# llGuy/madrona_renderer

Measured on AMD Instinct MI355X. Metric: rendered views/sec (whole node), N worlds x 64x64 RGB+depth, higher is better.
Workload: dtype f32

## Files before the change

madrona_renderer_amd/csrc/raster.hip:

```cpp
#include <hip/hip_runtime.h>
#include <algorithm>
#include <cstdlib>

#include "raster.hpp"
#include "raster_dev.hpp"

namespace mrx {
namespace {

constexpr int kWavesPerBlock = 4;
constexpr int kChunk = 64;
constexpr int kHot = 16;
constexpr int kBandRows = 16;
constexpr int kBlocksPerBand = 16;

struct WaveLds {
    float hot[kChunk][kHot];
    float cold[kChunk][kCold];
};

struct TileCtx {
    uint32_t view, tileX0, tileY0;
    uint32_t triBegin, numTris;
    int lx, ly;
// ... 185 lines not shown
                    resolvePixel<IDS>(p, L, bid[b], best[b], pxf[b & 7],
                                      (b >> 3) ? py1 : py0, outRgba[b], outId[b]);
        } else {
            for (uint32_t chunk = 0; chunk < t.numTris; chunk += kChunk) {
                const uint64_t mask = setupChunk<PV>(p, vc, t, chunk, lane, L, pr, lt);
                rasterBandBrute(L, mask, pxf, py0, py1, invNear, best, bid);
#pragma unroll
                for (int b = 0; b < kBlocksPerBand; ++b) {
                    if (bid[b] >= 0)
                        resolvePixel<IDS>(p, L, bid[b], best[b], pxf[b & 7],
                                          (b >> 3) ? py1 : py0, outRgba[b], outId[b]);
                    bid[b] = -1;
                }
                waveLdsSync();
            }
        }

#pragma unroll
        for (int b = 0; b < kBlocksPerBand; ++b) {
            const int r = b >> 3, bx = b & 7;
            const uint32_t fx = t.tileX0 + bx * 8 + t.lx;
            const uint32_t fy = t.tileY0 + band * kBandRows + r * 8 + t.ly;
            if (fx < p.nfast && fy < p.nslow) {
                const bool hit = best[b] > p.invFar;
                const float dep = hit ? 1.0f / best[b] : 0.0f;
                const size_t o = ((size_t)t.view * p.nslow + fy) * p.nfast + fx;
                if (storesRgb<OUT>(p.rgb))
                    p.rgb[o] = outRgba[b];
                if (storesDepth<OUT>(p.depth))
                    p.depth[o] = dep;
                if (IDS)
                    p.ids[o] = outId[b];
            }
        }
    }
}

template <bool IDS, bool MULTI, int OUT = kOutRGBD>
__global__ __launch_bounds__(kWave *kWavesPerBlock)
void rasterBruteKernel(const RasterParams p)
{
    bruteKernelBody<IDS, MULTI, OUT, false>(p);
}

template <bool IDS, bool MULTI>
__global__ __launch_bounds__(kWave *kWavesPerBlock)
void rasterBruteKernelPV(const RasterParams p)
{
    bruteKernelBody<IDS, MULTI, kOutByPointer, true>(p);
}

constexpr uint32_t kNearFree = 1u << 16;

template <int S0, int S1>
__device__ __forceinline__ uint32_t classifyStrips(const TriPlanes &c, uint32_t tileX0,
                                                   uint32_t tileY0, float invNear, float invFar,
                                                   bool &nearOk)
{
    const float X0 = (float)tileX0, Y0 = (float)tileY0;
    const float xa0 = c.A0 < 0.0f ? X0 : X0 + 31.0f;
    const float xa1 = c.A1 < 0.0f ? X0 : X0 + 31.0f;
    const float xa2 = c.A2 < 0.0f ? X0 : X0 + 31.0f;
    const float xdh = c.Dx < 0.0f ? X0 : X0 + 31.0f;
    const float xdl = c.Dx < 0.0f ? X0 + 31.0f : X0;
    const float yb0 = c.B0 < 0.0f ? Y0 : Y0 + 7.0f;
    const float yb1 = c.B1 < 0.0f ? Y0 : Y0 + 7.0f;
    const float yb2 = c.B2 < 0.0f ? Y0 : Y0 + 7.0f;
    const float ydh = c.Dy < 0.0f ? Y0 : Y0 + 7.0f;
    const float ydl = c.Dy < 0.0f ? Y0 + 7.0f : Y0;
    uint32_t mask = 0;
    float dmax = -__builtin_inff();
#pragma unroll
    for (int s = S0; s < S1; ++s) {
        const float dy = (float)(8 * s);
        const float r0 = __builtin_fmaf(c.B0, yb0 + dy, c.C0);
        const float r1 = __builtin_fmaf(c.B1, yb1 + dy, c.C1);
        const float r2 = __builtin_fmaf(c.B2, yb2 + dy, c.C2);
        const float rh = __builtin_fmaf(c.Dy, ydh + dy, c.Dc);
        const float rl = __builtin_fmaf(c.Dy, ydl + dy, c.Dc);
        const bool yin = (Y0 + dy + 7.0f >= c.bbY0) && (Y0 + dy <= c.bbY1);
#pragma unroll
        for (int hf = 0; hf < 2; ++hf) {
            const float dx = (float)(32 * hf);
            const float e0 = __builtin_fmaf(c.A0, xa0 + dx, r0);
            const float e1 = __builtin_fmaf(c.A1, xa1 + dx, r1);
            const float e2 = __builtin_fmaf(c.A2, xa2 + dx, r2);
            const float dh = __builtin_fmaf(c.Dx, xdh + dx, rh);
            const float dl = __builtin_fmaf(c.Dx, xdl + dx, rl);
            const bool xin = (X0 + dx + 31.0f >= c.bbX0) && (X0 + dx <= c.bbX1);
            const bool possible = (fminf(fminf(e0, e1), e2) >= 0.0f) &&
                                  (dh > invFar) && (dl <= invNear) && xin && yin;
            mask |= possible ? (1u << (2 * s + hf)) : 0u;
            dmax = fmaxf(dmax, dh);
        }
    }
    nearOk = dmax <= invNear;
    return mask;
}

__device__ __forceinline__ uint32_t classifyRegions(const TriPlanes &c, const TileCtx &t,
                                                    float invNear, float invFar)
{
    bool nearOk;
    uint32_t mask = classifyStrips<0, 8>(c, t.tileX0, t.tileY0, invNear, invFar, nearOk);
    if (nearOk)
        mask |= kNearFree;
    return mask;
}


template <bool NEAR>
__device__ __forceinline__ void pixelTest(const PlanePairs &q, f32x2 r01, f32x2 r2d, float px,
                                          float invNear, int32_t kv, float &best, int32_t &bid)
{
    const f32x2 pp = { px, px };
    const f32x2 e01 = fma2(q.A01, pp, r01);
    const f32x2 e2d = fma2(q.A2D, pp, r2d);
    bool in = (fminf(fminf(e01.x, e01.y), e2d.x) >= 0.0f) & (e2d.y > best);
    if (NEAR)
        in = in & (e2d.y <= invNear);
    best = in ? e2d.y : best;
    bid = in ? kv : bid;
}

template <bool NEAR, int IDSHIFT>
__device__ __forceinline__ void rasterRegion(const float (*planes)[16], uint64_t act, int recBase,
                                             const float (&px)[kRegionBlocks], float py,
                                             float invNear,
                                             float (&best)[kRegionBlocks],
                                             int32_t (&bid)[kRegionBlocks])
{
    const f32x2 yy = { py, py };
    for (; act != 0; act &= act - 1) {
        const int k = recBase + __builtin_ctzll(act);
        const PlanePairs q = loadPlanes(planes, k);
        const f32x2 r01 = fma2(q.B01, yy, q.C01);
        const f32x2 r2d = fma2(q.B2D, yy, q.C2D);
#pragma unroll
        for (int b = 0; b < kRegionBlocks; ++b)
            pixelTest<NEAR>(q, r01, r2d, px[b], invNear, k << IDSHIFT, best[b], bid[b]);
    }
}

template <bool IDS>
__device__ __forceinline__ void outputRegion(const RasterParams &p, const TileCtx &t,
                                             uint32_t fx0, uint32_t fy, float invFar,
                                             const float (&best)[kRegionBlocks],
                                             const uint32_t (&rgba)[kRegionBlocks],
                                             const int32_t (&id)[kRegionBlocks])
// ... 126 lines not shown
                                      outRgba[g][b], outId[g][b]);
                bid[g][b] = -1;
            }
        }
    }

#pragma unroll
    for (int g = 0; g < 4; ++g) {
        const int strip = 2 * wave + (g >> 1), hf = g & 1;
        const uint32_t fy = t.tileY0 + strip * 8 + t.ly;
        const uint32_t fx0 = t.tileX0 + hf * 32 + 4 * t.lx;
        outputRegion<IDS>(p, t, fx0, fy, invFar, best[g], outRgba[g], outId[g]);
    }
}

template <bool IDS>
__global__ __launch_bounds__(kWave *kWavesPerBlock, 3)
void rasterChunkedKernel(const RasterParams p)
{
    chunkedKernelBody<IDS, false>(p);
}

template <bool IDS>
__global__ __launch_bounds__(kWave *kWavesPerBlock, 3)
void rasterChunkedKernelPV(const RasterParams p)
{
    chunkedKernelBody<IDS, true>(p);
}

constexpr int kGroupTilesMax = 16;
constexpr int kGroupSlotsMax = 256;
constexpr int groupTilesMax(int slots) { return slots <= 128 ? kGroupTilesMax : 8; }

template <int SLOTS, bool PV = false>
struct GroupLds {
    static constexpr int kRecs = SLOTS <= kChunk ? kChunk + 16 : SLOTS;
    static constexpr int kBackground = kRecs;
    float planes[kRecs][16];
    uint32_t live[kRecs];
    float shade[kRecs + 1][4];
    float cold[kRecs][kCold];
    uint32_t masks[groupTilesMax(SLOTS) * (SLOTS <= kChunk ? kChunk : SLOTS)];
    uint32_t tileInfo[kGroupTilesMax][4];
    float tileNear[PV ? kGroupTilesMax : 1];
    uint32_t nextItem;
    uint8_t itemOrder[kGroupTilesMax * 8];
    uint2 items[SLOTS == 16 ? kGroupTilesMax * 8 : 1];
    uint8_t itemPos[SLOTS == 16 ? kGroupTilesMax * 8 : 1];
};
constexpr uint32_t kTileValid = 4u;
constexpr uint32_t kItemValid = 1u << 8;
constexpr uint32_t kItemNearFree = 1u << 9;
constexpr uint32_t kItemAnyTex = 1u << 10;


template <bool IDS, bool FULL, bool TEX, int OUT, typename LDS>
__device__ __forceinline__ void storeRegion(const RasterParams &p, const LDS &L, bool doRgb, bool doDepth,
                                            uint32_t *rgbTile, float *depthTile, int32_t *idsTile,
                                            uint32_t pixOff, uint32_t fx0, uint32_t fy,
                                            bool anyTex, const float (&px)[kRegionBlocks], float py,
                                            const float (&best)[kRegionBlocks],
                                            const int32_t (&bid)[kRegionBlocks])
{
    uint32_t rgba[kRegionBlocks];
    int32_t id[kRegionBlocks];
    float dep[kRegionBlocks];
    const char *shadeBase = reinterpret_cast<const char *>(&L.shade[0][0]);
#pragma unroll
    for (int b = 0; b < kRegionBlocks; ++b) {
        const float *h = reinterpret_cast<const float *>(shadeBase + bid[b]);
        if (OUT != kOutDepth)
            rgba[b] = __float_as_uint(h[0]);
        if (IDS)
            id[b] = __float_as_int(p.idsAreSegmask ? h[2] : h[3]);
        if (OUT != kOutRGB)
            dep[b] = bid[b] != LDS::kBackground * 16 ? __builtin_amdgcn_rcpf(best[b]) : 0.0f;
    }
    if (TEX && OUT != kOutDepth && anyTex && (OUT != kOutByPointer || doRgb)) {
#pragma unroll
        for (int b = 0; b < kRegionBlocks; ++b) {
            const int32_t rec = bid[b] >> 4;
            const int32_t tex = __float_as_int(L.shade[rec][1]);
            if (tex >= 0)
                rgba[b] = shadeTextured(p, L.cold[rec], tex, px[b], py, 1.0f / best[b]);
        }
    }
    if (p.debugSkip & 1u)
        return;
    if (FULL) {
        if (doRgb)
            streamStore16(p.writeThrough, rgbTile + pixOff, rgba[0], rgba[1], rgba[2], rgba[3]);
        if (doDepth)
            streamStore16(p.writeThrough, depthTile + pixOff, __float_as_uint(dep[0]), __float_as_uint(dep[1]),
                          __float_as_uint(dep[2]), __float_as_uint(dep[3]));
        if (IDS)
            streamStore16(p.writeThrough, idsTile + pixOff, (uint32_t)id[0], (uint32_t)id[1], (uint32_t)id[2], (uint32_t)id[3]);
    } else if (fy < p.nslow) {
#pragma unroll
        for (int b = 0; b < kRegionBlocks; ++b) {
            if (fx0 + b < p.nfast) {
                if (doRgb)
                    streamStore4(p.writeThrough, rgbTile + pixOff + b, rgba[b]);
                if (doDepth)
                    streamStore4(p.writeThrough, depthTile + pixOff + b, __float_as_uint(dep[b]));
                if (IDS)
                    streamStore4(p.writeThrough, idsTile + pixOff + b, (uint32_t)id[b]);
            }
        }
    }
}

template <bool IDS, bool FULL>
__device__ __forceinline__ void storeBackground(const RasterParams &p, bool doRgb, bool doDepth, uint32_t *rgbTile,
                                                float *depthTile, int32_t *idsTile,
                                                uint32_t pixOff, uint32_t fx0, uint32_t fy)
{
    if (p.debugSkip & 1u)
        return;
    const uint32_t bg = 0xFF000000u;
    if (FULL) {
        if (doRgb)
            streamStore16(p.writeThrough, rgbTile + pixOff, bg, bg, bg, bg);
        if (doDepth)
            streamStore16(p.writeThrough, depthTile + pixOff, 0u, 0u, 0u, 0u);
        if (IDS)
            streamStore16(p.writeThrough, idsTile + pixOff, ~0u, ~0u, ~0u, ~0u);
    } else if (fy < p.nslow) {
#pragma unroll
        for (int b = 0; b < kRegionBlocks; ++b) {
            if (fx0 + b < p.nfast) {
                if (doRgb)
                    streamStore4(p.writeThrough, rgbTile + pixOff + b, bg);
                if (doDepth)
                    streamStore4(p.writeThrough, depthTile + pixOff + b, 0u);
                if (IDS)
                    streamStore4(p.writeThrough, idsTile + pixOff + b, ~0u);
            }
        }
    }
}

template <typename LDS>
__device__ __forceinline__ uint32_t classifyPair(const LDS &L, int j, int k, int wave, float invNear, float invFar,
                                                 bool &nearOk, bool &tex)
{
    nearOk = false;
    tex = false;
    const uint32_t info = L.tileInfo[j][3];
    const int rec = (int)(info >> 8) + k;
    if (!(info & kTileValid) || !L.live[rec])
        return 0u;
    const float4 *src = reinterpret_cast<const float4 *>(L.planes[rec]);
    const float4 a = src[0], b = src[1], cc = src[2], bb = src[3];
    TriPlanes c;
    c.A0 = a.x; c.A1 = a.y; c.A2 = a.z; c.Dx = a.w;
    c.B0 = b.x; c.B1 = b.y; c.B2 = b.z; c.Dy = b.w;
    c.C0 = cc.x; c.C1 = cc.y; c.C2 = cc.z; c.Dc = cc.w;
    c.bbX0 = bb.x; c.bbX1 = bb.y; c.bbY0 = bb.z; c.bbY1 = bb.w;
    const uint32_t tx0 = L.tileInfo[j][1], ty0 = L.tileInfo[j][2];
    uint32_t m;
    switch (wave & 3) {
    case 0: m = classifyStrips<0, 2>(c, tx0, ty0, invNear, invFar, nearOk); break;
    case 1: m = classifyStrips<2, 4>(c, tx0, ty0, invNear, invFar, nearOk); break;
    case 2: m = classifyStrips<4, 6>(c, tx0, ty0, invNear, invFar, nearOk); break;
    default: m = classifyStrips<6, 8>(c, tx0, ty0, invNear, invFar, nearOk); break;
    }
    tex = __float_as_int(L.shade[rec][1]) >= 0;
    return m;
}

constexpr int groupWaves(bool tex) { return tex ? 4 : 8; }

template <bool IDS, int SLOTS, bool TEX, int XMODE, bool FAST, int OUT, bool PV = false, bool LT = false, bool COL = false,
          bool MAT = false>
__device__ __forceinline__ void groupKernelBody(const char *hPose, const char *hGeom, uint32_t hViews, uint32_t hInstances,
                                                uint32_t hPool, uint32_t hShape, uint32_t hGroups, uint32_t hPrefix,
                                                uint32_t hFirst01, uint32_t hFirst23, const RasterParams p)
{
    __shared__ GroupLds<SLOTS, PV> lds;
    constexpr int kBackground = GroupLds<SLOTS, PV>::kBackground;
    const int wave = __builtin_amdgcn_readfirstlane(threadIdx.x / kWave);
    const int lane = threadIdx.x % kWave;
    if (!FAST || wave >= 2)
        touchKernelArguments<(FAST ? 48 : 0) + sizeof(RasterParams)>();
    const uint32_t aNumViews = FAST ? hViews : p.numViews;
    const uint32_t aGrpViews = FAST ? (hShape & 255u) : p.grpViews;
    const uint32_t aXcdSkew = FAST ? ((hShape >> 8) & 15u) : p.xcdSkew;
    const uint32_t aXcdRotate = FAST ? ((hShape >> 12) & 1u) : p.xcdRotate;
    const uint32_t aGrpPerView = FAST ? 1u : p.grpPerView;
    const uint32_t aGrid = FAST ? hGroups : gridDim.x;
    const uint32_t aUniInstances = FAST ? ((hShape >> 13) & 7u) : p.uniInstances;
    const uint32_t aUniCams = FAST ? ((hShape >> 16) & 255u) : p.uniCamsPerWorld;
    const uint32_t dskip = FAST ? 0u : p.debugSkip;
    const PoseLayout lay = poseLayout(hViews, hInstances);
    const float *aCamRot = FAST ? reinterpret_cast<const float *>(hPose + lay.camRot) : p.camRot;
    const float *aCamPos = FAST ? reinterpret_cast<const float *>(hPose + lay.camPos) : p.camPos;
    const int32_t *aInstObj = FAST ? reinterpret_cast<const int32_t *>(hPose + lay.instObj) : p.instObj;
    const uint32_t *aInstColor = FAST ? reinterpret_cast<const uint32_t *>(hPose + lay.total)
                                 : MAT ? reinterpret_cast<const uint32_t *>(p.poseBlock + poseColorOffset(p.numViews, p.numInstances))
                                       : p.instColor;
    const int32_t *aInstMat = FAST ? reinterpret_cast<const int32_t *>(hPose + lay.total + mrxAlign256(hInstances * 4u))
                                   : p.instMat;
    const uint32_t tilesPerView = FAST ? 1u : p.tilesFast * p.tilesSlow;
    constexpr bool readyItems = FAST && !TEX;
    uint32_t firstView, groupViews, firstTile, groupTiles;
    const uint32_t blk = ((XMODE & 1) && SLOTS == 16 && aXcdSkew && (blockIdx.x ^ 1u) < aGrid)
                             ? blockIdx.x ^ 1u : blockIdx.x;
    if ((XMODE & 2) && blockIdx.x == 0 && threadIdx.x == (groupWaves(TEX) - 1) * kWave && p.xccReport)
        *p.xccReport = __builtin_amdgcn_s_getreg((3 << 11) | 20);
    uint32_t bid = blk;
    if (aXcdRotate && (bid | 7u) < aGrid)
        bid = (bid & ~7u) | ((bid + 2u * (bid >> 3)) & 7u);
    if (aGrpPerView == 1) {
        firstView = bid * aGrpViews;
        groupViews = aGrpViews;
        firstTile = 0;
        groupTiles = groupViews * tilesPerView;
    } else {
        firstView = bid / aGrpPerView;
        groupViews = 1;
        firstTile = (bid - firstView * aGrpPerView) * p.grpChunkTiles;
        groupTiles = min(p.grpChunkTiles, tilesPerView - firstTile);
    }
    uint32_t firstStrip = 0, numStrips = groupTiles * 8;
    if (SLOTS == 16 && aXcdSkew) {
        if (blk & 1u) {
            firstStrip = aXcdSkew;
            numStrips -= aXcdSkew;
        } else {
            groupViews += 1;
            groupTiles += 1;
            numStrips += aXcdSkew;
        }
    }
    const int groupRecs = (int)groupViews * SLOTS;
    const int numPairs = (int)groupTiles * SLOTS;
    const float invNear = p.invNear, invFar = p.invFar;
    if (dskip & 16u)
        return;
    unsigned long long *stamps = (!FAST && p.debugStamps && wave < 4)
        ? p.debugStamps + ((size_t)blockIdx.x * 4 + wave) * 8 : nullptr;
#define MRX_STAMP(i)                                                           \
    do {                                                                       \
        if (stamps && lane == 0)                                               \
            stamps[i] = __builtin_amdgcn_s_memrealtime();                      \
    } while (0)
    MRX_STAMP(0);
    if (!readyItems)
        for (int i = threadIdx.x; i < numPairs; i += groupWaves(TEX) * kWave)
            lds.masks[i] = 0u;

    if (wave == groupWaves(TEX) - 1 && lane < (int)groupTiles) {
        uint32_t vi = (uint32_t)lane, tile = firstTile;
        if (tilesPerView != 1) {
            vi = groupViews == 1 ? 0u : (uint32_t)lane / tilesPerView;
            tile = firstTile + (uint32_t)lane - vi * tilesPerView;
        }
// ... 66 lines not shown
#pragma unroll
            for (int r = 0; r < 3; ++r) {
                vc.c[r] = aCamPos[3 * view + r];
                vc.lv[r] = dot3(vc.Rc[0][r], vc.Rc[1][r], vc.Rc[2][r],
                                lt.toLight[0], lt.toLight[1], lt.toLight[2]);
            }
        }
        TriPlanes c;
        c.A0 = c.B0 = c.C0 = c.A1 = c.B1 = c.C1 = 0.0f;
        c.A2 = c.B2 = c.C2 = c.Dx = c.Dy = c.Dc = 0.0f;
        c.bbX0 = c.bbX1 = c.bbY0 = c.bbY1 = 0.0f;
        bool valid = false;
        MRX_STAMP(1);
        if (recOk) {
            lds.shade[rec][1] = __int_as_float(-1);
            if ((uint32_t)k < numTris && !(dskip & 8u)) {
                const ViewProj pr = viewProjOf(p, PV, view);
                const GroupSetupArgs sa = {
                    FAST ? reinterpret_cast<const ObjTri *>(hGeom) : p.tris,
                    FAST ? reinterpret_cast<const TriMat *>(hGeom + geomMatsOffset(hPool)) : p.triMats,
                    FAST ? reinterpret_cast<const float *>(hPose + lay.instPos) : p.instPos,
                    FAST ? reinterpret_cast<const float *>(hPose + lay.instRot) : p.instRot,
                    FAST ? reinterpret_cast<const float *>(hPose + lay.instScale) : p.instScale,
                    pr.sx, pr.ox, pr.sz, pr.oz, pr.s6bPad, lt.ambient, lt.diffuse, p.transposed };
                InstXform x;
                instanceTransform(sa, vc, wt.inst, x);
                const MatOverride mo = { MAT ? aInstMat[wt.inst] : -1, p.numMaterials, p.matTable };
                valid = setupTriangleCore<true, OUT != kOutDepth, COL, MAT>(sa, vc.lv, x, wt.tri, aInstObj[wt.inst], k, c,
                                                                            lds.shade[rec], lds.cold[rec],
                                                                            COL ? aInstColor[wt.inst] : 0u, mo);
            }
            MRX_STAMP(2);
            float4 *dst = reinterpret_cast<float4 *>(lds.planes[rec]);
            dst[0] = make_float4(c.A0, c.A1, c.A2, c.Dx);
            dst[1] = make_float4(c.B0, c.B1, c.B2, c.Dy);
            dst[2] = make_float4(c.C0, c.C1, c.C2, c.Dc);
            dst[3] = make_float4(c.bbX0, c.bbX1, c.bbY0, c.bbY1);
            lds.live[rec] = (valid && !(dskip & 4u)) ? 1u : 0u;
        }
        if (rec == 0) {
            lds.nextItem = 0;
            lds.shade[kBackground][0] = __uint_as_float(0xFF000000u);
            lds.shade[kBackground][1] = __int_as_float(-1);
            lds.shade[kBackground][2] = __int_as_float(-1);
            lds.shade[kBackground][3] = __int_as_float(-1);
        }
    }
    __syncthreads();
    MRX_STAMP(3);

    constexpr int kPairStride = (groupWaves(TEX) / 4) * kWave;
    for (int pair = (wave >> 2) * kWave + lane; pair - lane < numPairs; pair += kPairStride) {
        if (readyItems) {
            uint32_t m = 0;
            bool nearOk = false, tex = false;
            if (pair < numPairs)
                m = classifyPair(lds, pair / SLOTS, pair % SLOTS, wave, PV ? lds.tileNear[pair / SLOTS] : invNear, invFar,
                                 nearOk, tex);
            m >>= 4 * (wave & 3);
            const uint64_t l0 = __ballot(m & 1u), r0 = __ballot(m & 2u), l1 = __ballot(m & 4u), r1 = __ballot(m & 8u);
            const uint64_t near0 = __ballot((m & 3u) && !nearOk), near1 = __ballot((m & 12u) && !nearOk);
            const uint64_t tex0 = __ballot((m & 3u) && tex), tex1 = __ballot((m & 12u) && tex);
            if (lane % 16 == 0 && pair < numPairs) {
                const uint32_t j = (uint32_t)pair / 16u;
                const uint32_t valid = firstView + j < aNumViews ? kItemValid : 0u;
                const auto put = [&](uint32_t strip, uint64_t l, uint64_t r, uint64_t nearHit, uint64_t texHit) {
                    const uint32_t pos = lds.itemPos[j * 8u + strip];
                    if (pos == 0xFFu)
                        return;
                    const uint32_t desc = j | strip << 4 | valid |
                                          (((nearHit >> lane) & 0xFFFFu) == 0 ? kItemNearFree : 0u) |
                                          (((texHit >> lane) & 0xFFFFu) != 0 ? kItemAnyTex : 0u);
                    lds.items[pos] = make_uint2((uint32_t)((l >> lane) & 0xFFFFu) | (uint32_t)((r >> lane) & 0xFFFFu) << 16,
                                                desc);
                };
                put(2u * (wave & 3), l0, r0, near0, tex0);
                put(2u * (wave & 3) + 1u, l1, r1, near1, tex1);
            }
            continue;
        }
        if (pair >= numPairs)
            continue;
        bool nearOk, tex;
        uint32_t m = classifyPair(lds, pair / SLOTS, pair % SLOTS, wave, PV ? lds.tileNear[pair / SLOTS] : invNear,
                                  invFar, nearOk, tex);
        if (nearOk)
            m |= 1u << (16 + (wave & 3));
        if (m)
            atomicOr(&lds.masks[pair], m);
    }
    __syncthreads();
    MRX_STAMP(4);

    const int lx = lane & 7, ly = lane >> 3;
    const uint32_t laneOff = (uint32_t)ly * p.nfast + 4u * lx;
    int cachedTile = -1, recBase = 0;
    constexpr int SUBS = (SLOTS + kWave - 1) / kWave;
    constexpr int LANES = SLOTS < kWave ? SLOTS : kWave;
    uint32_t view = 0, tileX0 = 0, tileY0 = 0, mask[SUBS] = {};
    float pxTile[2][kRegionBlocks] = {};
    bool anyTex = false, nearFree = false, full = false;
    uint32_t *rgbTile = nullptr;
    float *depthTile = nullptr;
    int32_t *idsTile = nullptr;
    const bool doRgb = storesRgb<OUT>(p.rgb), doDepth = storesDepth<OUT>(p.depth);
    uint32_t itemMasks = 0;
    float tileNear = invNear;
    if (readyItems) {
        full = (p.nfast & 3u) == 0 && 64u <= p.nfast && 64u <= p.nslow;
#pragma unroll
        for (int hf = 0; hf < 2; ++hf)
#pragma unroll
            for (int b = 0; b < kRegionBlocks; ++b)
                pxTile[hf][b] = (float)(hf * 32 + 4 * lx + b);
    }
    for (;;) {
        uint32_t item = 0;
        if (lane == 0)
            item = atomicAdd(&lds.nextItem, 1u);
        item = __builtin_amdgcn_readfirstlane(item);
        if (item >= numStrips)
            break;
        int j, strip;
        if (readyItems) {
            const uint2 d = lds.items[item];
            itemMasks = __builtin_amdgcn_readfirstlane(d.x);
            const uint32_t desc = __builtin_amdgcn_readfirstlane(d.y);
            if (!(desc & kItemValid))
                continue;
            j = (int)(desc & 15u);
            strip = (int)((desc >> 4) & 7u);
            nearFree = (desc & kItemNearFree) != 0;
            anyTex = (desc & kItemAnyTex) != 0;
            recBase = j * SLOTS;
            if (PV)
                tileNear = __uint_as_float(__builtin_amdgcn_readfirstlane(__float_as_uint(lds.tileNear[j])));
            const size_t tileBase = (size_t)(firstView + (uint32_t)j) * p.nslow * p.nfast;
            rgbTile = p.rgb + tileBase;
            depthTile = p.depth + tileBase;
            idsTile = IDS ? p.ids + tileBase : nullptr;
        } else {
            item = __builtin_amdgcn_readfirstlane((uint32_t)lds.itemOrder[item]);
            j = (int)(item >> 3);
            strip = (int)(item & 7u);
            if (j != cachedTile) {
                const uint32_t info = __builtin_amdgcn_readfirstlane(lds.tileInfo[j][3]);
                if (!(info & kTileValid))
                    continue;
                cachedTile = j;
                recBase = (int)(info >> 8);
                view = __builtin_amdgcn_readfirstlane(lds.tileInfo[j][0]);
                tileX0 = __builtin_amdgcn_readfirstlane(lds.tileInfo[j][1]);
                tileY0 = __builtin_amdgcn_readfirstlane(lds.tileInfo[j][2]);
                if (PV)
                    tileNear = __uint_as_float(__builtin_amdgcn_readfirstlane(__float_as_uint(lds.tileNear[j])));
                const size_t tileBase = ((size_t)view * p.nslow + tileY0) * p.nfast + tileX0;
                rgbTile = p.rgb + tileBase;
                depthTile = p.depth + tileBase;
                idsTile = IDS ? p.ids + tileBase : nullptr;
                full = (p.nfast & 3u) == 0 && tileX0 + 64u <= p.nfast && tileY0 + 64u <= p.nslow;
                anyTex = false;
                nearFree = true;
#pragma unroll
                for (int sub = 0; sub < SUBS; ++sub) {
                    const int slot = sub * kWave + lane;
                    mask[sub] = lane < LANES ? lds.masks[j * SLOTS + slot] : 0u;
                    const int32_t tex = lane < LANES ? __float_as_int(lds.shade[recBase + slot][1]) : -1;
                    anyTex = anyTex || __ballot((mask[sub] & 0xFFFFu) != 0 && tex >= 0) != 0;
                    nearFree = nearFree &&
                               __ballot((mask[sub] & 0xFFFFu) != 0 && ((mask[sub] >> 16) & 0xFu) != 0xFu) == 0;
                }
#pragma unroll
                for (int hf = 0; hf < 2; ++hf)
#pragma unroll
                    for (int b = 0; b < kRegionBlocks; ++b)
                        pxTile[hf][b] = (float)(tileX0 + hf * 32 + 4 * lx + b);
            }
        }
        const uint32_t fy = tileY0 + strip * 8 + ly;
        const float py = (float)fy;
#pragma unroll
        for (int hf = 0; hf < 2; ++hf) {
            const uint32_t fx0 = tileX0 + hf * 32 + 4 * lx;
            const uint32_t pixOff = (uint32_t)(strip * 8) * p.nfast + hf * 32 + laneOff;
            uint64_t act[SUBS];
            bool any = false;
#pragma unroll
            for (int sub = 0; sub < SUBS; ++sub) {
                act[sub] = readyItems ? (uint64_t)((itemMasks >> (16 * hf)) & 0xFFFFu)
                                     : __ballot((mask[sub] >> (2 * strip + hf)) & 1u);
                any = any || act[sub] != 0;
            }
            if (!any) {
                if (full)
                    storeBackground<IDS, true>(p, doRgb, doDepth, rgbTile, depthTile, idsTile, pixOff, fx0, fy);
                else
                    storeBackground<IDS, false>(p, doRgb, doDepth, rgbTile, depthTile, idsTile, pixOff, fx0, fy);
                continue;
            }
            const float (&px)[kRegionBlocks] = pxTile[hf];
            float best[kRegionBlocks];
            int32_t bid[kRegionBlocks];
#pragma unroll
            for (int b = 0; b < kRegionBlocks; ++b) {
                best[b] = invFar;
                bid[b] = kBackground * 16;
            }
            if (!(dskip & 2u)) {
#pragma unroll
                for (int sub = 0; sub < SUBS; ++sub) {
                    if (SUBS > 1 && act[sub] == 0)
                        continue;
                    if (nearFree)
                        rasterRegion<false, 4>(lds.planes, act[sub], recBase + sub * kWave, px, py, tileNear, best, bid);
                    else
                        rasterRegion<true, 4>(lds.planes, act[sub], recBase + sub * kWave, px, py, tileNear, best, bid);
                }
            }
            if (full)
                storeRegion<IDS, true, TEX, OUT>(p, lds, doRgb, doDepth, rgbTile, depthTile, idsTile, pixOff, fx0, fy,
                                            anyTex, px, py, best, bid);
            else
                storeRegion<IDS, false, TEX, OUT>(p, lds, doRgb, doDepth, rgbTile, depthTile, idsTile, pixOff, fx0, fy,
                                             anyTex, px, py, best, bid);
        }
    }
    MRX_STAMP(5);
    MRX_STAMP(6);
    if (stamps && lane == 0)
        stamps[7] = ((unsigned long long)__builtin_amdgcn_s_getreg((31 << 11) | 20) << 32) |
                    (unsigned long long)__builtin_amdgcn_s_getreg((31 << 11) | 4);
#undef MRX_STAMP
}

template <bool IDS, int SLOTS, bool TEX, int XMODE = 0, int OUT = kOutRGBD>
__global__ __launch_bounds__(kWave *groupWaves(TEX), TEX ? (SLOTS > 128 ? 3 : 4) : (SLOTS > 128 ? 6 : 8))
void rasterGroupKernel(const RasterParams p)
{
    groupKernelBody<IDS, SLOTS, TEX, XMODE, false, OUT>(nullptr, nullptr, 0u, 0u, 0u, 0u, 0u, 0u, 0u, 0u, p);
}

template <bool IDS, bool TEX, int XMODE, int OUT>
__global__ __launch_bounds__(kWave *groupWaves(TEX), TEX ? 4 : 8)
void rasterGroupKernelFast(const char *hPose, const char *hGeom, uint32_t hViews, uint32_t hInstances, uint32_t hPool,
                           uint32_t hShape, uint32_t hGroups, uint32_t hPrefix, uint32_t hFirst01, uint32_t hFirst23,
                           const RasterParams p)
{
    groupKernelBody<IDS, 16, TEX, XMODE, true, OUT>(hPose, hGeom, hViews, hInstances, hPool, hShape, hGroups, hPrefix, hFirst01,
                                               hFirst23, p);
}
// ... 167 lines not shown
        if (tpv == 1) {
            vg = std::max<uint32_t>(1u, (uint32_t)(kChunk / slots));
            if (p.anyTextured)
                vg = std::min<uint32_t>(vg, 2u);
            while (vg > 1 && (p.numViews + vg - 1) / vg < (vg == 2 ? kFill / 2 : kFill))
                vg /= 2;
        } else if (p.anyTextured) {
            ct = std::max<uint32_t>(1u, std::min<uint32_t>(4u, tpv / 4u));
        } else {
            ct = std::min<uint32_t>(tpv, std::min<uint32_t>(maxTiles, 8u));
        }
        if (tpv != 1)
            while (ct > 1 && (uint64_t)p.numViews * ((tpv + ct - 1) / ct) < kFill)
                ct = (ct + 1) / 2;
        if (p.grpViewsWanted > 0 && tpv * (uint32_t)p.grpViewsWanted <= maxTiles &&
            p.grpViewsWanted * slots <= kChunk) {
            vg = (uint32_t)p.grpViewsWanted;
            ct = tpv;
        }
        if (p.grpTilesWanted > 0 && (uint32_t)p.grpTilesWanted <= maxTiles) {
            vg = 1;
            ct = std::min<uint32_t>((uint32_t)p.grpTilesWanted, tpv);
        }
        gpv = (tpv + ct - 1) / ct;
        q.grpViews = vg;
        q.grpChunkTiles = ct;
        q.grpPerView = gpv;
        const uint32_t numGroups = gpv == 1 ? (p.numViews + vg - 1) / vg : p.numViews * gpv;
        const bool skewable = slots == 16 && tpv == 1 && (vg == 4 || vg == 2);
        q.xcdSkew = (skewable && numGroups >= kFill) ? (vg == 4 ? 3u : 1u) : 0u;
        if (p.xcdSkewWanted >= 0)
            q.xcdSkew = skewable ? (uint32_t)(p.xcdSkewWanted < 8 ? p.xcdSkewWanted : 7) : 0u;
        q.xcdRotate = (tpv == 1 && numGroups >= kFill) ? 1u : 0u;
        if (p.xcdRotateWanted >= 0)
            q.xcdRotate = p.xcdRotateWanted ? 1u : 0u;
        const dim3 grid(numGroups);
        const dim3 gblock(kWave * groupWaves(p.anyTextured != 0));
        GroupHeader h {};
        h.pose = p.poseBlock;
        h.geom = p.geomBlock;
        h.views = p.numViews;
        h.instances = p.numInstances;
        h.poolTris = p.poolTris;
        h.groups = numGroups;
        bool fast = slots == 16 && tpv == 1 && gpv == 1 && p.uniInstances != 0 && p.uniCamsPerWorld < 256 && vg < 256 &&
                    p.poseBlock && p.geomBlock && p.debugSkip == 0 && p.debugStamps == nullptr && p.uniPrefix[4] < 256;
        for (int i = 0; i < 4 && fast; ++i)
            fast = p.uniFirstTri[i] < 65536u;
        if (const char *dbg = std::getenv("MRX_GROUP_FAST"))
            fast = fast && std::atoi(dbg) != 0;
        if (entry) *entry = fast ? kEntryGroupFast : kEntryGroup;
        if (fast) {
            h.shape = vg | (q.xcdSkew << 8) | (q.xcdRotate << 12) | (p.uniInstances << 13) | (p.uniCamsPerWorld << 16) | (1u << 31);
            h.prefix = p.uniPrefix[1] | (p.uniPrefix[2] << 8) | (p.uniPrefix[3] << 16) | (p.uniPrefix[4] << 24);
            h.first01 = p.uniFirstTri[0] | (p.uniFirstTri[1] << 16);
            h.first23 = p.uniFirstTri[2] | (p.uniFirstTri[3] << 16);
        }
#define MRX_GROUP_ARGS h.pose, h.geom, h.views, h.instances, h.poolTris, h.shape, h.groups, h.prefix, h.first01, h.first23, q
#define MRX_GROUP_FORM(S, FK, K)                                               \
    do {                                                                       \
        if (fast && S == 16) {                                                 \
            if (ids) { if (p.anyTextured) FK<true, true><<<grid, gblock, 0, stream>>>(MRX_GROUP_ARGS);    \
                       else FK<true, false><<<grid, gblock, 0, stream>>>(MRX_GROUP_ARGS); }               \
            else     { if (p.anyTextured) FK<false, true><<<grid, gblock, 0, stream>>>(MRX_GROUP_ARGS);   \
                       else FK<false, false><<<grid, gblock, 0, stream>>>(MRX_GROUP_ARGS); }              \
        } else if (ids) {                                                      \
            if (p.anyTextured) K<true, S, true><<<grid, gblock, 0, stream>>>(q);                          \
            else               K<true, S, false><<<grid, gblock, 0, stream>>>(q);                         \
        } else {                                                               \
            if (p.anyTextured) K<false, S, true><<<grid, gblock, 0, stream>>>(q);                         \
            else               K<false, S, false><<<grid, gblock, 0, stream>>>(q);                        \
        }                                                                      \
    } while (0)
#define MRX_GROUP_O(S, X, O, OP)                                               \
    do {                                                                       \
        if (p.instMat && pv && p.tablesVary) {                                 \
            MRX_GROUP_FORM(S, rasterGroupKernelFastPVLM, rasterGroupKernelPVLM);                          \
        } else if (p.instMat) {                                                \
            MRX_GROUP_FORM(S, rasterGroupKernelFastM, rasterGroupKernelM);     \
        } else if (p.instColor && pv && p.tablesVary) {                        \
            MRX_GROUP_FORM(S, rasterGroupKernelFastPVLC, rasterGroupKernelPVLC);                          \
        } else if (p.instColor) {                                              \
            MRX_GROUP_FORM(S, rasterGroupKernelFastC, rasterGroupKernelC);     \
        } else if (pv && p.lightTable) {                                       \
            MRX_GROUP_FORM(S, rasterGroupKernelFastPVL, rasterGroupKernelPVL); \
        } else if (pv) {                                                       \
            MRX_GROUP_FORM(S, rasterGroupKernelFastPV, rasterGroupKernelPV);   \
        } else if (fast && S == 16) {                                          \
            if (p.anyTextured) {                                               \
                if (ids) rasterGroupKernelFast<true, true, X, O><<<grid, gblock, 0, stream>>>(MRX_GROUP_ARGS);   \
                else     rasterGroupKernelFast<false, true, X, O><<<grid, gblock, 0, stream>>>(MRX_GROUP_ARGS);  \
            } else {                                                           \
                if (ids) rasterGroupKernelFast<true, false, X, O><<<grid, gblock, 0, stream>>>(MRX_GROUP_ARGS);  \
                else     rasterGroupKernelFast<false, false, X, O><<<grid, gblock, 0, stream>>>(MRX_GROUP_ARGS); \
            }                                                                  \
        } else if (p.anyTextured) {                                            \
            if (ids) rasterGroupKernel<true, S, true, X, OP><<<grid, gblock, 0, stream>>>(q);   \
            else     rasterGroupKernel<false, S, true, X, OP><<<grid, gblock, 0, stream>>>(q);  \
        } else {                                                               \
            if (ids) rasterGroupKernel<true, S, false, X, OP><<<grid, gblock, 0, stream>>>(q);  \
            else     rasterGroupKernel<false, S, false, X, OP><<<grid, gblock, 0, stream>>>(q); \
        }                                                                      \
    } while (0)
        const OutSel out = outSelOf(p.rgb, p.depth);
#define MRX_GROUP_X(S, X)                                                      \
    do {                                                                       \
// ... 27 lines not shown
```

madrona_renderer_amd/csrc/raster.hpp:

```cpp
#pragma once

#include <cstdint>
#include <hip/hip_runtime_api.h>

namespace mrx {

struct BvhNode;
struct ObjInfo;

struct alignas(32) ViewProj {
    float sx, ox, sz, oz;
    float invNear, s6bPad;
    float pad[2];
};
static_assert(sizeof(ViewProj) == 32, "ViewProj is one 32-byte record");

struct alignas(32) ViewLight {
    float toLight[3];
    float ambient, diffuse;
    float pad[3];
};
static_assert(sizeof(ViewLight) == 32, "ViewLight is one 32-byte record");

struct alignas(16) ObjTri {
// ... 82 lines not shown
    const ObjInfo *instInfo;
    uint32_t numObjects;
    uint32_t bvhUniInst, bvhUniCams;
    const uint32_t *worldInstStart;
    const uint32_t *viewWorld;
    const uint32_t *instKBase;
    uint32_t bvhPassInst;
    int32_t bvhTile;
    int32_t bvhSmallArea;
    int32_t bvhClassify;
    uint32_t bvhGroupTiles;
    uint32_t bvhGroupViews;
    uint32_t bvhFlat;
    uint32_t bvhTexCap;
    uint32_t numCUs;
    const ViewProj *viewProj;
    const ViewLight *viewLight;
    uint32_t lightTable;
    uint32_t tablesVary;
    const uint32_t *instColor;
    const int32_t *instMat;
    const MatRec *matTable;
    uint32_t numMaterials;
};

#if defined(__HIP__) || defined(__HIPCC__)
#define MRX_HD __host__ __device__
#else
#define MRX_HD
#endif
struct PoseLayout {
    uint32_t camRot, camPos, instRot, instPos, instScale, instObj, total;
};
MRX_HD inline uint32_t mrxAlign256(uint32_t x) { return (x + 255u) & ~255u; }
MRX_HD inline PoseLayout poseLayout(uint32_t views, uint32_t instances)
{
    PoseLayout l;
    l.camRot = 0;
    l.camPos = l.camRot + mrxAlign256(views * 16u);
    l.instRot = l.camPos + mrxAlign256(views * 12u);
    l.instPos = l.instRot + mrxAlign256(instances * 16u);
    l.instScale = l.instPos + mrxAlign256(instances * 12u);
    l.instObj = l.instScale + mrxAlign256(instances * 12u);
    l.total = l.instObj + mrxAlign256(instances * 4u);
    return l;
}
MRX_HD inline uint32_t poseColorOffset(uint32_t views, uint32_t instances) { return poseLayout(views, instances).total; }
MRX_HD inline uint32_t poseMaterialOffset(uint32_t views, uint32_t instances)
{
    return poseColorOffset(views, instances) + mrxAlign256(instances * 4u);
}
MRX_HD inline uint32_t geomMatsOffset(uint32_t poolTris) { return mrxAlign256(poolTris * 64u); }

struct GroupHeader {
    const char *pose;
    const char *geom;
    uint32_t views, instances, poolTris;
    uint32_t shape;
    uint32_t groups;
    uint32_t prefix;
    uint32_t first01, first23;
};

constexpr uint32_t kBvhMinTris = 129;

enum OutSel : int {
    kOutRGBD = 0,
    kOutDepth = 1,
    kOutRGB = 2,
    kOutByPointer = 3
};
inline OutSel outSelOf(const void *rgb, const void *depth)
{
    return !rgb ? kOutDepth : !depth ? kOutRGB : kOutRGBD;
}

enum KernelVariant : int32_t {
    kVariantDefault = 0,
    kVariantBrute = 1,
    kVariantBvh = 2,
    kVariantRaster = 3,
    kNumVariants
};

inline uint32_t groupFill(uint32_t numCUs) { return 4u * (numCUs ? numCUs : 256u); }
inline uint32_t bvhDispatchMinTris(uint32_t base, uint32_t numViews, bool anyTextured, uint32_t nfast, uint32_t nslow,
                                   uint32_t numCUs)
{
    const uint32_t cus = numCUs ? numCUs : 256u;
    if (nfast > 64u || nslow > 64u)
        return base;
    if (2ull * numViews <= 5ull * cus)
        return base < 65u ? base : 65u;
    if (numViews <= 4u * cus && !anyTextured)
        return base < 91u ? base : 91u;
    return base;
}

inline bool bvhDispatchFlat(bool raytracer, uint32_t numViews, uint32_t nfast, uint32_t nslow, uint32_t maxWorldTris,
                            uint32_t maxWorldInstances, uint32_t numCUs)
{
    const uint32_t cus = numCUs ? numCUs : 256u;
    const uint64_t tpv = (uint64_t)((nfast + 63u) / 64u) * ((nslow + 63u) / 64u);
    return raytracer && maxWorldTris >= 1u && maxWorldTris <= 64u && maxWorldInstances <= 64u && tpv >= 16u &&
           (uint64_t)numViews * tpv >= 192ull * cus;
}
// ... 21 lines not shown
```

Before: 186.2 million.

## Fast-path regions fully covered by a single triangle with uniform store

Extends the per-strip classification to also detect 32x8 regions that lie entirely inside one triangle's edges and depth range. It encodes per-region uniform flags into the work-item descriptor. In the shading phase, such regions bypass per-pixel triangle testing and write a constant color/id and plane-interpolated depth directly. This adds extra edge evaluations and ballots during classification, gated by an environment variable that defaults on.

```diff
diff --git a/madrona_renderer_amd/csrc/raster.hip b/madrona_renderer_amd/csrc/raster.hip
--- a/madrona_renderer_amd/csrc/raster.hip
+++ b/madrona_renderer_amd/csrc/raster.hip
@@ -261,10 +261,10 @@
 
 constexpr uint32_t kNearFree = 1u << 16;
 
-template <int S0, int S1>
+template <int S0, int S1, bool INSIDE = false>
 __device__ __forceinline__ uint32_t classifyStrips(const TriPlanes &c, uint32_t tileX0,
                                                    uint32_t tileY0, float invNear, float invFar,
-                                                   bool &nearOk)
+                                                   bool &nearOk, uint32_t *inside = nullptr)
 {
     const float X0 = (float)tileX0, Y0 = (float)tileY0;
     const float xa0 = c.A0 < 0.0f ? X0 : X0 + 31.0f;
@@ -277,7 +277,7 @@
     const float yb2 = c.B2 < 0.0f ? Y0 : Y0 + 7.0f;
     const float ydh = c.Dy < 0.0f ? Y0 : Y0 + 7.0f;
     const float ydl = c.Dy < 0.0f ? Y0 + 7.0f : Y0;
-    uint32_t mask = 0;
+    uint32_t mask = 0, ins = 0;
     float dmax = -__builtin_inff();
 #pragma unroll
     for (int s = S0; s < S1; ++s) {
@@ -301,9 +301,37 @@
                                   (dh > invFar) && (dl <= invNear) && xin && yin;
             mask |= possible ? (1u << (2 * s + hf)) : 0u;
             dmax = fmaxf(dmax, dh);
+            if (INSIDE)
+                ins |= (possible && (dl > invFar) && (dh <= invNear)) ? (1u << (2 * s + hf)) : 0u;
         }
     }
     nearOk = dmax <= invNear;
+    if (INSIDE) {
+        __builtin_amdgcn_sched_barrier(0);
+        const float xi0 = c.A0 < 0.0f ? X0 + 31.0f : X0;
+        const float xi1 = c.A1 < 0.0f ? X0 + 31.0f : X0;
+        const float xi2 = c.A2 < 0.0f ? X0 + 31.0f : X0;
+        const float yi0 = c.B0 < 0.0f ? Y0 + 7.0f : Y0;
+        const float yi1 = c.B1 < 0.0f ? Y0 + 7.0f : Y0;
+        const float yi2 = c.B2 < 0.0f ? Y0 + 7.0f : Y0;
+#pragma unroll
+        for (int s = S0; s < S1; ++s) {
+            const float dy = (float)(8 * s);
+            const float q0 = __builtin_fmaf(c.B0, yi0 + dy, c.C0);
+            const float q1 = __builtin_fmaf(c.B1, yi1 + dy, c.C1);
+            const float q2 = __builtin_fmaf(c.B2, yi2 + dy, c.C2);
+#pragma unroll
+            for (int hf = 0; hf < 2; ++hf) {
+                const float dx = (float)(32 * hf);
+                const float i0 = __builtin_fmaf(c.A0, xi0 + dx, q0);
+                const float i1 = __builtin_fmaf(c.A1, xi1 + dx, q1);
+                const float i2 = __builtin_fmaf(c.A2, xi2 + dx, q2);
+                const bool whole = (i0 >= 0.0f) && (i1 >= 0.0f) && (i2 >= 0.0f);
+                ins &= whole ? ~0u : ~(1u << (2 * s + hf));
+            }
+        }
+        *inside = ins;
+    }
     return mask;
 }
 
@@ -536,6 +564,7 @@
 constexpr uint32_t kItemValid = 1u << 8;
 constexpr uint32_t kItemNearFree = 1u << 9;
 constexpr uint32_t kItemAnyTex = 1u << 10;
+constexpr uint32_t kItemUniformShift = 11;
 
 
 template <bool IDS, bool FULL, bool TEX, int OUT, typename LDS>
@@ -624,12 +653,38 @@
     }
 }
 
-template <typename LDS>
+template <bool IDS, int OUT, typename LDS>
+__device__ __forceinline__ void storeUniform(const RasterParams &p, const LDS &L, bool doRgb, bool doDepth,
+                                             uint32_t *rgbTile, float *depthTile, int32_t *idsTile,
+                                             uint32_t pixOff, int k, const float (&px)[kRegionBlocks], float py)
+{
+    const float *pl = L.planes[k];
+    const float *h = L.shade[k];
+    if (OUT != kOutDepth && doRgb) {
+        const uint32_t rgba = __float_as_uint(h[0]);
+        streamStore16(p.writeThrough, rgbTile + pixOff, rgba, rgba, rgba, rgba);
+    }
+    if (OUT != kOutRGB && doDepth) {
+        const float r = __builtin_fmaf(pl[7], py, pl[11]);
+        uint32_t dep[kRegionBlocks];
+#pragma unroll
+        for (int b = 0; b < kRegionBlocks; ++b)
+            dep[b] = __float_as_uint(__builtin_amdgcn_rcpf(__builtin_fmaf(pl[3], px[b], r)));
+        streamStore16(p.writeThrough, depthTile + pixOff, dep[0], dep[1], dep[2], dep[3]);
+    }
+    if (IDS) {
+        const uint32_t id = __float_as_uint(p.idsAreSegmask ? h[2] : h[3]);
+        streamStore16(p.writeThrough, idsTile + pixOff, id, id, id, id);
+    }
+}
+
+template <bool INSIDE, typename LDS>
 __device__ __forceinline__ uint32_t classifyPair(const LDS &L, int j, int k, int wave, float invNear, float invFar,
-                                                 bool &nearOk, bool &tex)
+                                                 bool &nearOk, bool &tex, uint32_t &inside)
 {
     nearOk = false;
     tex = false;
+    inside = 0u;
     const uint32_t info = L.tileInfo[j][3];
     const int rec = (int)(info >> 8) + k;
     if (!(info & kTileValid) || !L.live[rec])
@@ -641,13 +696,13 @@
     c.B0 = b.x; c.B1 = b.y; c.B2 = b.z; c.Dy = b.w;
     c.C0 = cc.x; c.C1 = cc.y; c.C2 = cc.z; c.Dc = cc.w;
     c.bbX0 = bb.x; c.bbX1 = bb.y; c.bbY0 = bb.z; c.bbY1 = bb.w;
-    const uint32_t tx0 = L.tileInfo[j][1], ty0 = L.tileInfo[j][2];
+    const uint32_t tx0 = INSIDE ? 0u : L.tileInfo[j][1], ty0 = INSIDE ? 0u : L.tileInfo[j][2];
     uint32_t m;
     switch (wave & 3) {
-    case 0: m = classifyStrips<0, 2>(c, tx0, ty0, invNear, invFar, nearOk); break;
-    case 1: m = classifyStrips<2, 4>(c, tx0, ty0, invNear, invFar, nearOk); break;
-    case 2: m = classifyStrips<4, 6>(c, tx0, ty0, invNear, invFar, nearOk); break;
-    default: m = classifyStrips<6, 8>(c, tx0, ty0, invNear, invFar, nearOk); break;
+    case 0: m = classifyStrips<0, 2, INSIDE>(c, tx0, ty0, invNear, invFar, nearOk, &inside); break;
+    case 1: m = classifyStrips<2, 4, INSIDE>(c, tx0, ty0, invNear, invFar, nearOk, &inside); break;
+    case 2: m = classifyStrips<4, 6, INSIDE>(c, tx0, ty0, invNear, invFar, nearOk, &inside); break;
+    default: m = classifyStrips<6, 8, INSIDE>(c, tx0, ty0, invNear, invFar, nearOk, &inside); break;
     }
     tex = __float_as_int(L.shade[rec][1]) >= 0;
     return m;
@@ -687,6 +742,7 @@
                                    : p.instMat;
     const uint32_t tilesPerView = FAST ? 1u : p.tilesFast * p.tilesSlow;
     constexpr bool readyItems = FAST && !TEX;
+    constexpr bool uniformRegions = readyItems && !LT;
     uint32_t firstView, groupViews, firstTile, groupTiles;
     const uint32_t blk = ((XMODE & 1) && SLOTS == 16 && aXcdSkew && (blockIdx.x ^ 1u) < aGrid)
                              ? blockIdx.x ^ 1u : blockIdx.x;
@@ -859,38 +915,44 @@
     constexpr int kPairStride = (groupWaves(TEX) / 4) * kWave;
     for (int pair = (wave >> 2) * kWave + lane; pair - lane < numPairs; pair += kPairStride) {
         if (readyItems) {
-            uint32_t m = 0;
+            uint32_t m = 0, ins = 0;
             bool nearOk = false, tex = false;
             if (pair < numPairs)
-                m = classifyPair(lds, pair / SLOTS, pair % SLOTS, wave, PV ? lds.tileNear[pair / SLOTS] : invNear, invFar,
-                                 nearOk, tex);
+                m = classifyPair<uniformRegions>(lds, pair / SLOTS, pair % SLOTS, wave, PV ? lds.tileNear[pair / SLOTS] : invNear,
+                                       invFar, nearOk, tex, ins);
             m >>= 4 * (wave & 3);
-            const uint64_t l0 = __ballot(m & 1u), r0 = __ballot(m & 2u), l1 = __ballot(m & 4u), r1 = __ballot(m & 8u);
-            const uint64_t near0 = __ballot((m & 3u) && !nearOk), near1 = __ballot((m & 12u) && !nearOk);
-            const uint64_t tex0 = __ballot((m & 3u) && tex), tex1 = __ballot((m & 12u) && tex);
-            if (lane % 16 == 0 && pair < numPairs) {
-                const uint32_t j = (uint32_t)pair / 16u;
-                const uint32_t valid = firstView + j < aNumViews ? kItemValid : 0u;
-                const auto put = [&](uint32_t strip, uint64_t l, uint64_t r, uint64_t nearHit, uint64_t texHit) {
-                    const uint32_t pos = lds.itemPos[j * 8u + strip];
-                    if (pos == 0xFFu)
-                        return;
-                    const uint32_t desc = j | strip << 4 | valid |
-                                          (((nearHit >> lane) & 0xFFFFu) == 0 ? kItemNearFree : 0u) |
-                                          (((texHit >> lane) & 0xFFFFu) != 0 ? kItemAnyTex : 0u);
-                    lds.items[pos] = make_uint2((uint32_t)((l >> lane) & 0xFFFFu) | (uint32_t)((r >> lane) & 0xFFFFu) << 16,
-                                                desc);
-                };
-                put(2u * (wave & 3), l0, r0, near0, tex0);
-                put(2u * (wave & 3) + 1u, l1, r1, near1, tex1);
+            ins = (uniformRegions && (hShape & kShapeUniformRegions)) ? ins >> 4 * (wave & 3) : 0u;
+            const bool leader = lane % 16 == 0 && pair < numPairs;
+            const uint32_t j = (uint32_t)pair / 16u;
+            const uint32_t valid = firstView + j < aNumViews ? kItemValid : 0u;
+#pragma unroll
+            for (uint32_t i = 0; i < 2u; ++i) {
+                const uint32_t mi = m >> 2 * i, wi = ins >> 2 * i;
+                const uint64_t l = __ballot(mi & 1u), r = __ballot(mi & 2u);
+                const uint64_t il = __ballot(wi & 1u), ir = __ballot(wi & 2u);
+                const uint64_t nearHit = __ballot((mi & 3u) && !nearOk), texHit = __ballot((mi & 3u) && tex);
+                if (!leader)
+                    continue;
+                const uint32_t strip = 2u * (wave & 3) + i;
+                const uint32_t pos = lds.itemPos[j * 8u + strip];
+                if (pos == 0xFFu)
+                    continue;
+                const uint32_t lm = (uint32_t)((l >> lane) & 0xFFFFu), rm = (uint32_t)((r >> lane) & 0xFFFFu);
+                const uint32_t uniL = lm != 0 && (lm & (lm - 1u)) == 0 && (uint32_t)((il >> lane) & 0xFFFFu) == lm ? 1u : 0u;
+                const uint32_t uniR = rm != 0 && (rm & (rm - 1u)) == 0 && (uint32_t)((ir >> lane) & 0xFFFFu) == rm ? 2u : 0u;
+                const uint32_t desc = j | strip << 4 | valid | (uniL | uniR) << kItemUniformShift |
+                                      (((nearHit >> lane) & 0xFFFFu) == 0 ? kItemNearFree : 0u) |
+                                      (((texHit >> lane) & 0xFFFFu) != 0 ? kItemAnyTex : 0u);
+                lds.items[pos] = make_uint2(lm | rm << 16, desc);
             }
             continue;
         }
         if (pair >= numPairs)
             continue;
         bool nearOk, tex;
-        uint32_t m = classifyPair(lds, pair / SLOTS, pair % SLOTS, wave, PV ? lds.tileNear[pair / SLOTS] : invNear,
-                                  invFar, nearOk, tex);
+        uint32_t ins;
+        uint32_t m = classifyPair<false>(lds, pair / SLOTS, pair % SLOTS, wave, PV ? lds.tileNear[pair / SLOTS] : invNear,
+                                         invFar, nearOk, tex, ins);
         if (nearOk)
             m |= 1u << (16 + (wave & 3));
         if (m)
@@ -912,6 +974,7 @@
     int32_t *idsTile = nullptr;
     const bool doRgb = storesRgb<OUT>(p.rgb), doDepth = storesDepth<OUT>(p.depth);
     uint32_t itemMasks = 0;
+    uint32_t itemUniform = 0;
     float tileNear = invNear;
     if (readyItems) {
         full = (p.nfast & 3u) == 0 && 64u <= p.nfast && 64u <= p.nslow;
@@ -939,6 +1002,7 @@
             strip = (int)((desc >> 4) & 7u);
             nearFree = (desc & kItemNearFree) != 0;
             anyTex = (desc & kItemAnyTex) != 0;
+            itemUniform = uniformRegions && full ? (desc >> kItemUniformShift) & 3u : 0u;
             recBase = j * SLOTS;
             if (PV)
                 tileNear = __uint_as_float(__builtin_amdgcn_readfirstlane(__float_as_uint(lds.tileNear[j])));
@@ -1003,6 +1067,11 @@
                     storeBackground<IDS, true>(p, doRgb, doDepth, rgbTile, depthTile, idsTile, pixOff, fx0, fy);
                 else
                     storeBackground<IDS, false>(p, doRgb, doDepth, rgbTile, depthTile, idsTile, pixOff, fx0, fy);
+                continue;
+            }
+            if (uniformRegions && ((itemUniform >> hf) & 1u)) {
+                storeUniform<IDS, OUT>(p, lds, doRgb, doDepth, rgbTile, depthTile, idsTile, pixOff,
+                                       recBase + __builtin_ctz((uint32_t)act[0]), pxTile[hf], py);
                 continue;
             }
             const float (&px)[kRegionBlocks] = pxTile[hf];
@@ -1276,6 +1345,9 @@
         if (entry) *entry = fast ? kEntryGroupFast : kEntryGroup;
         if (fast) {
             h.shape = vg | (q.xcdSkew << 8) | (q.xcdRotate << 12) | (p.uniInstances << 13) | (p.uniCamsPerWorld << 16) | (1u << 31);
+            const char *uni = std::getenv("MRX_UNIFORM_REGIONS");
+            if (!uni || std::atoi(uni) != 0)
+                h.shape |= kShapeUniformRegions;
             h.prefix = p.uniPrefix[1] | (p.uniPrefix[2] << 8) | (p.uniPrefix[3] << 16) | (p.uniPrefix[4] << 24);
             h.first01 = p.uniFirstTri[0] | (p.uniFirstTri[1] << 16);
             h.first23 = p.uniFirstTri[2] | (p.uniFirstTri[3] << 16);
diff --git a/madrona_renderer_amd/csrc/raster.hpp b/madrona_renderer_amd/csrc/raster.hpp
--- a/madrona_renderer_amd/csrc/raster.hpp
+++ b/madrona_renderer_amd/csrc/raster.hpp
@@ -158,6 +158,7 @@
 }
 MRX_HD inline uint32_t geomMatsOffset(uint32_t poolTris) { return mrxAlign256(poolTris * 64u); }
 
+constexpr uint32_t kShapeUniformRegions = 1u << 24;
 struct GroupHeader {
     const char *pose;
     const char *geom;
```

Result: no change. 185.5 million (-0.4%).
